# raw-lab/mercat2

Measured on AMD Instinct MI355X. Metric: bases/sec at k=31, 10Mx150bp, higher is better.
Workload: dtype u64

## Files before the change

mercat2_amd/csrc/mk_skmer.hip:

```cpp
#include "mk_skmer_dev.h"
#include <cstdlib>
#include <cstdio>
#include <vector>
#include <type_traits>

#define SK_NKMAX 8
#ifndef SK_HIST_THREADS
#define SK_HIST_THREADS 256
#endif
#ifndef SK_HIST_GRID
#define SK_HIST_GRID 512
#endif
#ifndef SK_SCAT_GRID
#define SK_SCAT_GRID 4096
#endif
#define SK_MAX_P1_LOG2 13
#define SK_MAX_P1 (1 << SK_MAX_P1_LOG2)
#ifndef SK_BUCKET_SYMS
#define SK_BUCKET_SYMS 8192
#endif
#define SK_NOFIT 0xFF000000u

template <int W, class F>
__device__ __forceinline__ void sk_for_each_record(u64 w0, u64 w1, u64 badw, int k, int nkmax, bool canon, F&& emit) {
  const SkRuns r = sk_analyse<W>(w0, w1, sk_valid32(badw, k), canon);
  sk_walk(r, w0, w1, nkmax, canon, emit);
}

__device__ __forceinline__ ulonglong2 sk_make_record(u64 w0, u64 w1, int jstart, int nk, int k) {
  const int s = 2 * jstart;
  u64 hi = (w0 << s) | ((w1 >> 1) >> (63 - s));
  u64 lo = w1 << s;
  const int t = 2 * (nk + k - 1);
  const u64 mh = t >= 64 ? ~0ull : (~0ull << ((64 - t) & 63));
  const u64 ml = t <= 64 ? 0ull : (~0ull << ((128 - t) & 63));
  hi &= mh;
  lo = (lo & ml) | (u64)nk;
  return make_ulonglong2(hi, lo);
}

template <int W, bool CANON>
__global__ __launch_bounds__(SK_HIST_THREADS) void mk_sk_hist_k(const u64* __restrict__ codes, const u64* __restrict__ bad,
                                                                const MkChunkInfo* __restrict__ info, u64* __restrict__ hist,
                                                                u64* __restrict__ khist, int p1_log2, int k, int nkmax,
                                                                size_t nthreads_total, int canon, int sample_log2) {
  extern __shared__ unsigned sk_hist_lds[];
  (void)canon;
  sk_hist_body(sk_hist_lds, sk_hist_lds + (1u << p1_log2), info, hist, p1_log2, nthreads_total, sample_log2,
               [&](size_t t, size_t p0, auto&& tally) {
                 sk_for_each_record<W>(codes[t], codes[t + 1], bad_window(bad, p0), k, nkmax, CANON, tally);
               });
}

#ifndef SK_TU_CANON
__device__ __forceinline__ u64 sk_cap(u64 h, int sample_log2, u64 weight, float sigmas) {
  if (sample_log2 == 0) return h;
  const u64 est = h << sample_log2;
  const float dev = sigmas * __builtin_sqrtf((float)((u64)weight << sample_log2) * (float)est);
  return est + (u64)dev + 1 + (sigmas > 0 ? 16 * weight : 0);
}
__device__ __forceinline__ u64 sk_seg_cap(u64 h, int sample_log2, u64 weight, float sigmas, int nseg) {
  const float est = (float)(h << sample_log2);
  const float var = (float)weight * est * (1.0f / (float)nseg + (float)(1u << sample_log2) / (float)(nseg * nseg));
  return (u64)(est / (float)nseg) + (u64)(sigmas * __builtin_sqrtf(var)) + 1 + (sigmas > 0 ? 4 * weight : 0);
}
__global__ __launch_bounds__(1024) void mk_sk_scan_k(const u64* __restrict__ hist, const u64* __restrict__ khist,
                                                     u64* __restrict__ start, SkCursor* __restrict__ cursor, u64* __restrict__ kstart,
                                                     MkChunkInfo* __restrict__ info, int p1_log2, int sample_log2, int nkmax,
                                                     u64 div, u64 part_cap, u64 surv_cap, float sigmas, int nseg) {
  constexpr int PER = SK_MAX_P1 / 1024;
  __shared__ u64 wsum[16], wksum[16];
  const unsigned p1 = 1u << p1_log2;
  const unsigned per = (p1 + 1023) / 1024;
  const unsigned lo = threadIdx.x * per;
  const int lane = threadIdx.x & 63, wv = threadIdx.x >> 6;
  u64 cap[PER], kcap[PER];
  u64 acc = 0, kacc = 0;
#pragma unroll
  for (int q = 0; q < PER; ++q) {
    const unsigned i = lo + q;
    const bool on = (unsigned)q < per && i < p1;
    const u64 hk = on ? hist[i] : 0ull;
    cap[q] = !on ? 0 : (nseg > 1 ? sk_seg_cap(hk & 0xFFFFFFFFull, sample_log2, SK_R / SK_NKMAX, sigmas, 8)
                                 : sk_cap(hk & 0xFFFFFFFFull, sample_log2, SK_R / SK_NKMAX, sigmas));
    kcap[q] = on ? (sk_cap(hk >> 32, sample_log2, SK_R, sigmas) + div - 1) / div : 0;
    acc += cap[q];
    kacc += kcap[q];
  }
  u64 inc = acc, kinc = kacc;
#pragma unroll
  for (int d = 1; d < 64; d <<= 1) {
    const u64 a = __shfl_up(inc, d), b = __shfl_up(kinc, d);
    if (lane >= d) { inc += a; kinc += b; }
  }
  if (lane == 63) { wsum[wv] = inc; wksum[wv] = kinc; }
  __syncthreads();
  u64 run = inc - acc, krun = kinc - kacc;
  for (int w = 0; w < wv; ++w) { run += wsum[w]; krun += wksum[w]; }
  __shared__ u64 s_total;
  if (threadIdx.x == 1023) {
    const u64 total = run + acc, ktotal = krun + kacc;
    s_total = total;
    const u64 all = nseg > 1 ? 16 * total : total;
    start[(size_t)nseg * p1] = all;
    kstart[p1] = ktotal;
    if (all > part_cap) atomicOr(&info->part_overflow, 1ull);
    if (ktotal > surv_cap) atomicOr(&info->part_overflow, 2ull);
  }
  __shared__ unsigned s_run[SK_MAX_P1];
#pragma unroll
  for (int q = 0; q < PER; ++q) {
    const unsigned i = lo + q;
    if ((unsigned)q < per && i < p1) {
      s_run[i] = (unsigned)run;
      kstart[i] = krun;
      run += cap[q];
      krun += kcap[q];
    }
  }
  __syncthreads();
  const u64 total = s_total;
  for (int x = 0; x < nseg; ++x)
    for (unsigned i = threadIdx.x; i < p1; i += 1024) {
      const u64 at = x < 8 ? (u64)x * total + s_run[i] : 8 * total + 8 * (u64)s_run[i];
      start[(size_t)x * p1 + i] = at;
      cursor[(size_t)x * p1 + i] = (SkCursor)at;
    }
}

#endif

#ifdef MK_STAMP
static __device__ u64 skq_dbg[1024 * 8];
#endif
#define SKQ_CAP 512
#if defined(SK_ABL_COARSE) && !defined(SK_PLAIN_CURSORS)
#error "SK_ABL_COARSE needs -DSK_PLAIN_CURSORS (the ablation's region ends differ from the ones sk_reserve8k checks)"
#endif
#ifndef SKQ_THREADS
#define SKQ_THREADS 512
#endif
#define SKQ_WAVES (SKQ_THREADS / 64)
#define SKQ_WALKED 0xFFFFFFFFu
template <int W, bool CANON, int SKQ_SUBT, int SKQ_QCAP>
__global__ __launch_bounds__(SKQ_THREADS) __attribute__((amdgpu_waves_per_eu(4, 4))) void mk_sk_scatterq_k(const u64* __restrict__ codes, const u64* __restrict__ bad,
                                                         MkChunkInfo* __restrict__ info, const u64* __restrict__ start,
                                                         SkCursor* __restrict__ cursor, ulonglong2* __restrict__ part,
                                                         int p1_log2, int k, int nkmax, size_t ntiles, unsigned qcap, int nseg) {
  SkCursor* const shared_cursor = cursor + ((size_t)8 << p1_log2);
  const u64* const shared_start = start + ((size_t)8 << p1_log2);
  if (nseg > 1) {
    unsigned xcc;
    asm volatile("s_getreg_b32 %0, hwreg(HW_REG_XCC_ID)" : "=s"(xcc));
    const size_t seg = xcc & 7u;
    cursor += seg << p1_log2;
    start += seg << p1_log2;
  }
  __shared__ unsigned lh[SK_MAX_P1];
  __shared__ u64 pk_x[SKQ_SUBT][SKQ_WAVES][65];
  __shared__ unsigned queue[SKQ_SUBT][SKQ_WAVES][SKQ_QCAP];
  __shared__ unsigned s_abort;
  if (threadIdx.x == 0) s_abort = info->part_overflow != 0;
  __syncthreads();
  if (s_abort) return;
  unsigned spilled = 0;
  constexpr int NB = SK_MAX_P1 / SKQ_THREADS;
  const unsigned p1 = 1u << p1_log2;
  const size_t seq_len = info->seq_len;
  const int lane = threadIdx.x & 63;
#define wv sk_wave_id()
  auto sk_wave_id = [&]() { int w = (int)threadIdx.x; asm volatile("" : "+v"(w)); return w >> 6; };
  for (unsigned i = threadIdx.x; i < p1; i += blockDim.x) lh[i] = 0;
  __syncthreads();
  u64 tA = 0, tB = 0, tC = 0, tD = 0, tE = 0, tF = 0, t0 = 0, ntile = 0;
  (void)tA; (void)tB; (void)tC; (void)tD; (void)tE; (void)tF; (void)t0; (void)ntile;
  STAMP(t0);
  for (size_t tile = blockIdx.x; tile < ntiles; tile += gridDim.x) {
    ntile += 1;
    unsigned qn[SKQ_SUBT];
#pragma unroll
    for (int st = 0; st < SKQ_SUBT; ++st) {
      const size_t t = (tile * SKQ_SUBT + st) * SKQ_THREADS + threadIdx.x;
      const size_t p0 = t * SK_R;
      SkRuns runs;
      runs.valid = 0;
      runs.starts = 0;
      runs.pos[0] = runs.pos[1] = runs.pos[2] = runs.pos[3] = 0;
      u64 ww0 = 0, ww1 = 0;
      if (p0 < seq_len) {
        ww0 = codes[t];
        ww1 = codes[t + 1];
        runs = sk_analyse<W>(ww0, ww1, sk_valid32(bad_window(bad, p0), k), CANON);
      } else if (p0 < seq_len + SK_R) {
        ww0 = codes[t];
      }
      pk_x[st][wv][lane] = ww0;
      if (lane == 63) pk_x[st][wv][64] = ww1;
      const unsigned s2 = sk_cut_starts(runs.starts, runs.valid, nkmax);
      const unsigned cnt = __popc(s2);
      const unsigned inc = mk_wave_scan_incl(cnt);
      const unsigned total = mk_wave_last(inc);
      unsigned* const myq = queue[st][wv];
      if (total <= qcap) {
        unsigned todo = s2, at = inc - cnt;
        while (todo) {
          const int j = __ffs(todo) - 1;
          todo &= todo - 1;
          const unsigned stop = (s2 | ~runs.valid) & ~((2u << j) - 1);
          const int nk = (stop ? (__ffs(stop) - 1) : SK_R) - j;
          const u64 pw = j < 10 ? runs.pos[0] : (j < 20 ? runs.pos[1] : (j < 30 ? runs.pos[2] : runs.pos[3]));
          const unsigned best = (unsigned)(pw >> (6 * (j % 10))) & 63u;
          myq[at++] = (unsigned)lane | ((unsigned)j << 6) | ((unsigned)nk << 11) | (best << 16);
        }
        __builtin_amdgcn_fence(__ATOMIC_RELEASE, "wavefront");
        __builtin_amdgcn_wave_barrier();
        __builtin_amdgcn_fence(__ATOMIC_ACQUIRE, "wavefront");
        for (unsigned base = 0; base < total; base += 64) {
          const unsigned i = base + lane;
          if (i < total) {
            const unsigned it = myq[i];
            const u64* const wp = &pk_x[st][wv][it & 63u];
            const unsigned mm = sk_canon_mmer(sk_mmer(wp[0], wp[1], (int)(it >> 16)), CANON);
#ifdef SK_ABL_COARSE
            const unsigned b = sk_bucket(mm, p1_log2) & ~63u;
#else
            const unsigned b = sk_bucket(mm, p1_log2);
#endif
            atomicAdd(&lh[b], 1u);
            myq[i] = (it & 0xFFFFu) | (b << 16);
          }
        }
        qn[st] = total;
      } else {
        if (p0 < seq_len)
          sk_walk(runs, ww0, ww1, nkmax, CANON, [&](int, int, unsigned mm) {
            atomicAdd(&lh[sk_bucket(mm, p1_log2)], 1u);
          });
        qn[st] = SKQ_WALKED;
      }
    }
    STAMP_ADD(tA, t0);
    __syncthreads();
    STAMP_ADD(tB, t0);
    unsigned roff = 0;
    asm volatile("" : "+s"(roff));
    SkCursor* const rcursor = cursor + roff;
    const u64* const rstart = start + roff;
    SkCursor* const rshared_cursor = shared_cursor + roff;
    const u64* const rshared_start = shared_start + roff;
#ifndef SK_PLAIN_CURSORS
    if (p1 == SK_MAX_P1) {
      static_assert(NB % 8 == 0, "sk_reserve8");
#pragma unroll
      for (int h = 0; h < NB; h += 8) {
        unsigned v[8], at[8];
#pragma unroll
        for (int i = 0; i < 8; ++i) v[i] = lh[threadIdx.x + (h + i) * SKQ_THREADS];
        unsigned nofit = sk_reserve8<SKQ_THREADS>(v, rcursor + h * SKQ_THREADS, rstart + h * SKQ_THREADS, SK_NOFIT, at);
        if (nseg > 1 && __any(nofit)) {
          unsigned v2[8], at2[8];
#pragma unroll
          for (int i = 0; i < 8; ++i) {
            v2[i] = at[i] >= SK_NOFIT ? v[i] : 0u;
            const unsigned pad = at[i] >= SK_NOFIT ? at[i] & 0xFFFFFFu : 0u;
            if (pad) {
              const u64 end = rstart[threadIdx.x + (h + i) * SKQ_THREADS + 1];
              for (unsigned q = 0; q < pad; ++q) part[end - pad + q] = make_ulonglong2(0, 0);
            }
          }
          nofit = sk_reserve8<SKQ_THREADS>(v2, rshared_cursor + h * SKQ_THREADS, rshared_start + h * SKQ_THREADS, SK_NOFIT, at2);
#pragma unroll
          for (int i = 0; i < 8; ++i) at[i] = v2[i] ? at2[i] : at[i];
        }
        spilled |= nofit;
#pragma unroll
        for (int i = 0; i < 8; ++i) lh[threadIdx.x + (h + i) * SKQ_THREADS] = at[i];
      }
    } else
#endif
    {
      for (unsigned b = threadIdx.x; b < p1; b += SKQ_THREADS) {
        const unsigned v = lh[b];
        u64 r = v ? (u64)atomicAdd(&rcursor[b], v) : 0ull;
#ifdef SK_ABL_COARSE
        const bool fits = v == 0 || r + v <= rstart[b + 64 < p1 ? b + 64 : p1];
#else
        bool fits = v == 0 || r + v <= rstart[b + 1];
        if (!fits && nseg > 1) {
          for (u64 q = r; q < rstart[b + 1]; ++q) part[q] = make_ulonglong2(0, 0);
          r = (u64)atomicAdd(&rshared_cursor[b], v);
          fits = r + v <= rshared_start[b + 1];
        }
#endif
        spilled |= fits ? 0u : 1u;
        lh[b] = fits ? (unsigned)r : SK_NOFIT;
      }
    }
    STAMP_ADD(tC, t0);
    __syncthreads();
    STAMP_ADD(tD, t0);
#pragma unroll
    for (int st = 0; st < SKQ_SUBT; ++st) {
      if (qn[st] != SKQ_WALKED) {
        const unsigned total = qn[st];
        const unsigned* const myq = queue[st][wv];
        for (unsigned base = 0; base < total; base += 64) {
          const unsigned i = base + lane;
          if (i < total) {
            const unsigned it = myq[i];
            const unsigned at = atomicAdd(&lh[it >> 16], 1u);
            const u64* const wp = &pk_x[st][wv][it & 63u];
            ulonglong2 rec = sk_make_record(wp[0], wp[1], (int)((it >> 6) & 31u), (int)((it >> 11) & 31u), k);
            asm volatile("" : "+v"(rec.x), "+v"(rec.y));
            if (at < SK_NOFIT) part[(size_t)at] = rec;
          }
        }
      } else {
        const size_t t = (tile * SKQ_SUBT + st) * SKQ_THREADS + threadIdx.x;
        const size_t p0 = t * SK_R;
        if (p0 < seq_len) {
          const ulonglong2 w = make_ulonglong2(pk_x[st][wv][lane], pk_x[st][wv][lane + 1]);
          const SkRuns runs = sk_analyse<W>(w.x, w.y, sk_valid32(bad_window(bad, p0), k), CANON);
          sk_walk(runs, w.x, w.y, nkmax, CANON, [&](int jstart, int nk, unsigned mm) {
            const unsigned at = atomicAdd(&lh[sk_bucket(mm, p1_log2)], 1u);
            if (at < SK_NOFIT) part[(size_t)at] = sk_make_record(w.x, w.y, jstart, nk, k);
          });
        }
      }
    }
    STAMP_ADD(tE, t0);
    __syncthreads();
    for (unsigned i = threadIdx.x; i < p1; i += blockDim.x) lh[i] = 0;
    __syncthreads();
    STAMP_ADD(tF, t0);
  }
#ifdef MK_STAMP
  if (threadIdx.x == 0 && blockIdx.x < 1024) { u64* d = skq_dbg + (size_t)blockIdx.x * 8; d[0] = tA; d[1] = tB; d[2] = tC; d[3] = tD; d[4] = tE; d[5] = tF; d[6] = ntile; }
#endif
  if (spilled) atomicOr(&info->part_overflow, 4ull);
}
#undef wv


#ifndef SK_TU_CANON
void mk_launch_sk_scan(mk_ctx* c, const u64* hist, const u64* khist, u64* start, SkCursor* cursor, u64* kstart, int p1_log2,
                       int sample_log2, int nkmax, u64 surv_div, u64 part_cap, u64 surv_cap, float sigmas, int nseg) {
  hipLaunchKernelGGL(mk_sk_scan_k, dim3(1), dim3(1024), 0, c->stream, hist, khist, start, cursor, kstart,
                     (MkChunkInfo*)c->info.p, p1_log2, sample_log2, nkmax, surv_div, part_cap, surv_cap, sigmas, nseg);
}

#endif

template <int W, bool CANON>
static void launch_wc(mk_ctx* c, size_t seq_len, int p1_log2, int nkmax, int sample_log2, u64 surv_div, u64 part_cap, u64 surv_cap,
                     u64* hist, u64* start, SkCursor* cursor, u64* khist, u64* kstart, bool reuse, int nseg) {
  MkChunkInfo* info = (MkChunkInfo*)c->info.p;
  const size_t threads = div_up(seq_len, SK_R);
  const size_t tiles = div_up(div_up(threads, (size_t)1 << sample_log2), SK_HIST_THREADS);
  const size_t hist_grid = sample_log2 ? SK_HIST_GRID / 2 : SK_HIST_GRID;
  if (!reuse) {
    const float sigmas = (float)mk_env_double("MK_SAMPLE_SIGMAS", 6.0);
    hipLaunchKernelGGL((mk_sk_hist_k<W, CANON>), dim3((unsigned)(tiles < hist_grid ? tiles : hist_grid)), dim3(SK_HIST_THREADS),
                       2 * sizeof(unsigned) << p1_log2, c->stream,
                       (const u64*)c->codes.p, (const u64*)c->bad.p, info, hist, khist, p1_log2, c->k, nkmax, threads, c->canonical,
                       sample_log2);
    mk_launch_sk_scan(c, (const u64*)hist, (const u64*)khist, start, cursor, kstart, p1_log2, sample_log2, nkmax, surv_div, part_cap,
                      surv_cap, sigmas, nseg);
  }
  const SkQueueShape shape = sk_queue_shape(c);
  const bool three = shape.three;
  const unsigned qcap = shape.qcap;
  const size_t qtiles = div_up(threads, (size_t)SKQ_THREADS * (three ? 3 : 2));
  const dim3 qgrid((unsigned)(qtiles < SK_SCAT_GRID ? qtiles : SK_SCAT_GRID));
  if (three)
    hipLaunchKernelGGL((mk_sk_scatterq_k<W, CANON, 3, 376>), qgrid, dim3(SKQ_THREADS), 0, c->stream, (const u64*)c->codes.p,
                       (const u64*)c->bad.p, info, (const u64*)start, cursor, (ulonglong2*)c->part.p, p1_log2, c->k, nkmax, qtiles, qcap, nseg);
  else
    hipLaunchKernelGGL((mk_sk_scatterq_k<W, CANON, 2, 512>), qgrid, dim3(SKQ_THREADS), 0, c->stream, (const u64*)c->codes.p,
                       (const u64*)c->bad.p, info, (const u64*)start, cursor, (ulonglong2*)c->part.p, p1_log2, c->k, nkmax, qtiles, qcap, nseg);
#ifdef MK_STAMP
  {
    (void)hipStreamSynchronize(c->stream);
    const unsigned g = qgrid.x;
    std::vector<u64> h(8 * 1024);
    (void)hipMemcpyFromSymbol(h.data(), HIP_SYMBOL(skq_dbg), h.size() * 8);
    double a[7] = {0, 0, 0, 0, 0, 0, 0};
    for (unsigned w = 0; w < g && w < 1024; ++w) for (int q = 0; q < 7; ++q) a[q] += (double)h[w * 8 + q] / g;
    fprintf(stderr, "[stamp scatterq] per WG (wave 0): analyse+list+pass1=%.0f barrier1=%.0f cursors=%.0f barrier2=%.0f pass2=%.0f barrier3+clear=%.0f tiles=%.2f grid=%u\n",
            a[0], a[1], a[2], a[3], a[4], a[5], a[6], g);
  }
#endif
}


template <bool CANON>
static bool sk_partition(int W, mk_ctx* c, size_t seq_len, int p1_log2, int nkmax, int sample_log2, u64 surv_div, u64 part_cap, u64 surv_cap,
                         u64* hist, u64* start, SkCursor* cursor, u64* khist, u64* kstart, bool reuse, int nseg) {
  switch (W) {
#define SK_CASE(W_)                                                                                                      \
  case W_: launch_wc<W_, CANON>(c, seq_len, p1_log2, nkmax, sample_log2, surv_div, part_cap, surv_cap, hist, start, cursor, khist, kstart, reuse, nseg); return true;
    SK_CASE(2) SK_CASE(3) SK_CASE(4) SK_CASE(5) SK_CASE(6) SK_CASE(7)
    SK_CASE(8) SK_CASE(9) SK_CASE(10) SK_CASE(11) SK_CASE(12) SK_CASE(13) SK_CASE(14) SK_CASE(15) SK_CASE(16)
    SK_CASE(17) SK_CASE(18) SK_CASE(19) SK_CASE(20) SK_CASE(21) SK_CASE(22)
#undef SK_CASE
    default: return false;
  }
}

#ifdef SK_TU_CANON
bool mk_sk_partition_canon(int W, mk_ctx* c, size_t seq_len, int p1_log2, int nkmax, int sample_log2, u64 surv_div, u64 part_cap,
                           u64 surv_cap, u64* hist, u64* start, SkCursor* cursor, u64* khist, u64* kstart, bool reuse, int nseg) {
  return sk_partition<true>(W, c, seq_len, p1_log2, nkmax, sample_log2, surv_div, part_cap, surv_cap, hist, start, cursor, khist, kstart, reuse, nseg);
}
#else
bool mk_sk_partition_canon(int W, mk_ctx* c, size_t seq_len, int p1_log2, int nkmax, int sample_log2, u64 surv_div, u64 part_cap,
                           u64 surv_cap, u64* hist, u64* start, SkCursor* cursor, u64* khist, u64* kstart, bool reuse, int nseg);

bool mk_part_inherit(mk_ctx* c, size_t seq_len, int p1_log2, uint64_t min_count, bool sampled, bool exact) {
  if (c->part_cooldown > 0 && !exact) c->part_cooldown -= 1;
  const bool reuse = !exact && sampled && c->part_reuse_ok && !c->part_dirty && c->part_cooldown == 0 &&
                     p1_log2 == c->part_prev_p1 && (unsigned long long)min_count == c->part_prev_minc &&
                     seq_len <= c->part_prev_len + c->part_prev_len / 100 && seq_len >= c->part_prev_len - c->part_prev_len / 50 &&
                     !mk_env_set("MK_NO_REUSE");
  if (reuse) c->st.part_reused += 1;
  c->part_dirty = true;
  if (exact) { c->part_reuse_ok = false; c->part_cooldown = 4; }
  else if (sampled && !reuse) {
    c->part_reuse_ok = true;
    c->part_prev_len = seq_len;
    c->part_prev_p1 = p1_log2;
    c->part_prev_minc = (unsigned long long)min_count;
  } else if (!reuse) c->part_reuse_ok = false;
  return reuse;
}

int sk_p1_log2(size_t seq_len, int max_log2, size_t bucket_syms) {
  int p1_log2 = 8;
  while (p1_log2 < max_log2 && (seq_len >> p1_log2) > bucket_syms) ++p1_log2;
  return p1_log2;
}
int sk_sample_log2(size_t seq_len, bool exact) {
  return !exact && seq_len >= (size_t)mk_env_int("MK_SAMPLE_MIN", (long long)8 << 20) ? 3 : 0;
}
u64 sk_surv_div(uint64_t min_count) { return min_count > 1 ? (u64)min_count : 1; }
size_t sk_surv_cap(size_t seq_len, size_t p1, u64 surv_div, int sample_log2) {
  if (!sample_log2) return seq_len / surv_div + p1 + 64;
  const double L = 1.25 * (double)seq_len, S = (double)(1u << sample_log2), w = (double)SK_R;
  return (size_t)((L + 6.0 * sqrt((double)p1 * S * w * L) + 16.0 * w * (double)p1) / (double)surv_div) + 2 * p1 + 64;
}
SkQueueShape sk_queue_shape(const mk_ctx* c) {
  const long long force_subt = mk_env_int("MK_SKQ_SUBT", 0);
  SkQueueShape q;
  q.three = force_subt == 3 || (force_subt != 2 && c->items_hint > 0 && c->items_hint * 64.0 + 48.0 < 376.0);
  q.qcap = q.three ? 376u : 512u;
  { const long long v = mk_env_int("MK_SKQ_CAP", -1); if (v >= 0 && (unsigned long long)v < q.qcap) q.qcap = (unsigned)v; }
  return q;
}

int mk_launch_count_superkmer(mk_ctx* c, size_t seq_len, uint64_t min_count, bool exact) {
  if (seq_len == 0) return MK_OK;
  const int k = c->k;
  const int p1_log2 = sk_p1_log2(seq_len, SK_MAX_P1_LOG2, SK_BUCKET_SYMS);
  c->p1_log2 = p1_log2;
  const size_t p1 = (size_t)1 << p1_log2;
  int nkmax = 62 - k;
  if (nkmax > SK_NKMAX) nkmax = SK_NKMAX;
  { const long long v = mk_env_int("MK_NKMAX", 0); if (v >= 1 && v <= 31 && v <= 62 - k) nkmax = (int)v; }
  const int sample_log2 = sk_sample_log2(seq_len, exact);
  c->part_sampled = sample_log2 != 0;
  const int nseg = (sample_log2 != 0 && seq_len <= ((size_t)1 << 30) && mk_env_int("MK_XSEG", 1) != 0) ? 9 : 1;
  if (nseg != c->part_nseg) c->part_reuse_ok = false;
  c->part_nseg = nseg;
  const bool reuse = mk_part_inherit(c, seq_len, p1_log2, min_count, sample_log2 != 0, exact);
  int rc;
  if ((rc = mk_buf_reserve(c, c->part_meta, sk_meta_words(p1, SKC_SEG_MAX) * sizeof(u64))) != MK_OK) return rc;
  const size_t part_cap = nseg > 1 ? 2 * seq_len + 64 : seq_len + 64;
  if ((rc = mk_buf_reserve(c, c->part, part_cap * sizeof(ulonglong2))) != MK_OK) return rc;
  const u64 surv_div = sk_surv_div(min_count);
  const size_t surv_cap = sk_surv_cap(seq_len, p1, surv_div, sample_log2);
  if ((rc = mk_buf_reserve(c, c->surv_keys, surv_cap * sizeof(u64))) != MK_OK) return rc;
  if ((rc = mk_buf_reserve(c, c->surv_cnts, surv_cap * sizeof(u64))) != MK_OK) return rc;
  const SkMeta m = sk_meta(c->part_meta.p, p1, nseg);
  if (!reuse) MK_HIP(hipMemsetAsync(m.hist, 0, sk_meta_cleared_words(p1) * sizeof(u64), c->stream));
  mk_prof_begin(c, MK_K_PART);
  if (c->canonical) {
    if (!mk_sk_partition_canon(k - SK_M + 1, c, seq_len, p1_log2, nkmax, sample_log2, surv_div, (u64)part_cap, (u64)surv_cap, m.hist, m.start, m.cursor, m.khist, m.kstart, reuse, nseg)) {
      c->err = "mk_launch_count_superkmer: k out of range";
      return MK_ERR_ARG;
    }
  } else if (!sk_partition<false>(k - SK_M + 1, c, seq_len, p1_log2, nkmax, sample_log2, surv_div, (u64)part_cap, (u64)surv_cap, m.hist, m.start, m.cursor, m.khist, m.kstart, reuse, nseg)) {
    c->err = "mk_launch_count_superkmer: k out of range";
    return MK_ERR_ARG;
  }
  mk_prof_end(c);
  if ((rc = mk_launch_sk_count(c, (const u64*)m.start, m.cursor, (const u64*)m.kstart, m.nsurv, min_count, p1, nseg)) != MK_OK) return rc;
  MK_HIP(hipGetLastError());
  c->surv_regions = 1;
  return MK_OK;
}
#endif
```

mercat2_amd/csrc/mk_skmer_dev.h:

```cpp
#pragma once
#include "mk_common.h"
#include "mk_device.h"

#define SK_M 11
#define SK_MASK ((1u << (2 * SK_M)) - 1)
#define SK_R 32

__device__ __forceinline__ unsigned sk_order_raw(unsigned mm) {
  return __umul24(mm, 0x9277B5u) + 0x2C5A3Du;
}
__device__ __forceinline__ unsigned sk_order_hash(unsigned mm) { return sk_order_raw(mm) & SK_MASK; }
__device__ __forceinline__ unsigned sk_canon_mmer(unsigned mm, bool canon) {
  if (!canon) return mm;
  const unsigned rc = (unsigned)mk_revcomp2((u64)mm, SK_M);
  return rc < mm ? rc : mm;
}
__device__ __forceinline__ unsigned sk_bucket(unsigned mm, int p1_log2) { return (mm * 0xC2B2AE3Du) >> (32 - p1_log2); }

__device__ __forceinline__ unsigned sk_mmer(u64 w0, u64 w1, int q) {
  const u64 a = q < 32 ? w0 : w1, b = q < 32 ? w1 : 0ull;
  const int s = 2 * (q & 31);
  const u64 x = (a << s) | ((b >> 1) >> (63 - s));
  return (unsigned)(x >> (64 - 2 * SK_M));
}

typedef unsigned SkCursor;

#ifndef SK_PLAIN_CURSORS
template <int THREADS>
__device__ __forceinline__ unsigned sk_reserve8(const unsigned (&count)[8], SkCursor* cursor, const u64* start, unsigned nofit,
                                                unsigned (&base)[8]) {
  unsigned r[8];
  u64 lim[8];
  const unsigned voff4 = threadIdx.x * 4u, voff8 = threadIdx.x * 8u;
#pragma unroll
  for (int i = 0; i < 8; ++i) {
    u64 saved;
    r[i] = 0;
    asm volatile(
        "v_cmp_ne_u32 vcc, 0, %3\n\t"
        "s_and_saveexec_b64 %1, vcc\n\t"
        "s_nop 4\n\t"
        "global_atomic_add %0, %2, %3, %4 sc0\n\t"
        "s_mov_b64 exec, %1"
        : "+v"(r[i]), "=&s"(saved)
        : "v"(voff4), "v"(count[i]), "s"(cursor + i * THREADS)
        : "memory", "vcc", "scc");
  }
#pragma unroll
  for (int i = 0; i < 8; ++i)
    asm volatile("s_nop 4\n\tglobal_load_dwordx2 %0, %1, %2 offset:8" : "=&v"(lim[i]) : "v"(voff8), "s"(start + i * THREADS) : "memory");
  asm volatile("s_waitcnt vmcnt(0)"
               : "+v"(r[0]), "+v"(r[1]), "+v"(r[2]), "+v"(r[3]), "+v"(r[4]), "+v"(r[5]), "+v"(r[6]), "+v"(r[7]), "+v"(lim[0]),
                 "+v"(lim[1]), "+v"(lim[2]), "+v"(lim[3]), "+v"(lim[4]), "+v"(lim[5]), "+v"(lim[6]), "+v"(lim[7])
               :
               : "memory");
  unsigned spilled = 0;
#pragma unroll
  for (int i = 0; i < 8; ++i) {
    const bool fits = count[i] == 0 || (u64)r[i] + count[i] <= lim[i];
    spilled |= fits ? 0u : 1u;
    base[i] = fits ? r[i] : nofit | ((u64)r[i] < lim[i] ? (unsigned)(lim[i] - r[i]) : 0u);
  }
  return spilled;
}
#endif

template <int THREADS, int MAX_P1>
__device__ __forceinline__ void sk_reserve_tile(unsigned* count, unsigned* base, SkCursor* cursor, const u64* start, unsigned p1,
                                                unsigned nofit, unsigned& spilled) {
#ifndef SK_PLAIN_CURSORS
  if (p1 == MAX_P1) {
    constexpr int NB = MAX_P1 / THREADS;
    static_assert(NB % 8 == 0, "sk_reserve8");
#pragma unroll
    for (int h = 0; h < NB; h += 8) {
      unsigned v[8], at[8];
#pragma unroll
      for (int i = 0; i < 8; ++i) v[i] = count[threadIdx.x + (h + i) * THREADS];
      spilled |= sk_reserve8<THREADS>(v, cursor + h * THREADS, start + h * THREADS, nofit, at);
#pragma unroll
      for (int i = 0; i < 8; ++i) {
        base[threadIdx.x + (h + i) * THREADS] = at[i];
        if (base != count) count[threadIdx.x + (h + i) * THREADS] = 0;
      }
    }
  } else
#endif
  {
    for (unsigned b = threadIdx.x; b < p1; b += THREADS) {
      const unsigned v = count[b];
      const u64 r = v ? (u64)atomicAdd(&cursor[b], v) : 0ull;
      const bool fits = v == 0 || r + v <= start[b + 1];
      spilled |= fits ? 0u : 1u;
      base[b] = fits ? (unsigned)r : nofit;
      if (base != count) count[b] = 0;
    }
  }
}

__device__ __forceinline__ unsigned sk_valid32(u64 badw, int k) {
  if (badw == 0) return ~0u;
  u64 d = badw;
  int cover = 1;
  while (2 * cover <= k) { d |= d >> cover; cover *= 2; }
  if (cover < k) d |= d >> (k - cover);
  return ~(unsigned)d;
}

struct SkRuns {
  unsigned valid, starts;
  u64 pos[4];
};

template <int W>
__device__ __forceinline__ SkRuns sk_analyse(u64 w0, u64 w1, unsigned valid, bool canon) {
  constexpr int NQ = SK_R + W - 1;
  unsigned ord[NQ];
  {
    unsigned mm = sk_mmer(w0, w1, 0);
#pragma unroll
    for (int q = 0; q < NQ; ++q) {
      if (q) {
        const int pos = q + SK_M - 1;
        const unsigned base = (unsigned)((pos < 32 ? (w0 >> (62 - 2 * pos)) : (w1 >> (62 - 2 * (pos - 32)))) & 3u);
        mm = ((mm << 2) | base) & SK_MASK;
      }
      unsigned h = sk_order_raw(sk_canon_mmer(mm, canon));
      asm("" : "+v"(h));
      ord[q] = (h << 10) | (unsigned)q;
    }
  }
  constexpr int WA = W >= 3 ? 3 : 1, WB = W >= 9 ? 9 : WA;
  if constexpr (W >= 3) {
#pragma unroll
    for (int q = 0; q + 2 < NQ; ++q) ord[q] = min(min(ord[q], ord[q + 1]), ord[q + 2]);
  }
  if constexpr (W >= 9) {
#pragma unroll
    for (int q = 0; q + 8 < NQ; ++q) ord[q] = min(min(ord[q], ord[q + 3]), ord[q + 6]);
  }
  static_assert(W <= 3 * WB, "a third round of minima would be needed");
  SkRuns r;
  r.valid = valid;
  r.starts = 0;
  r.pos[0] = r.pos[1] = r.pos[2] = r.pos[3] = 0;
  unsigned prev_pos = 64;
#pragma unroll
  for (int j = 0; j < SK_R; ++j) {
    const bool ok = (valid >> j) & 1u;
    unsigned best;
    if constexpr (W == WB) best = ord[j];
    else if constexpr (W <= 2 * WB) best = min(ord[j], ord[j + W - WB]);
    else best = min(min(ord[j], ord[j + WB]), ord[j + W - WB]);
    best &= 63u;
    r.starts |= (ok && best != prev_pos) ? (1u << j) : 0u;
    prev_pos = ok ? best : 64u;
    r.pos[j / 10] |= (u64)best << (6 * (j % 10));
  }
  return r;
}

template <class F>
__device__ __forceinline__ void sk_walk(const SkRuns& r, u64 w0, u64 w1, int nkmax, bool canon, F&& emit) {
  unsigned todo = r.starts;
  while (todo) {
    const int j = __ffs(todo) - 1;
    todo &= todo - 1;
    const unsigned stop = (r.starts | ~r.valid) & ~((2u << j) - 1);
    int nk = (stop ? (__ffs(stop) - 1) : SK_R) - j;
    const u64 pw = j < 10 ? r.pos[0] : (j < 20 ? r.pos[1] : (j < 30 ? r.pos[2] : r.pos[3]));
    const unsigned best = (unsigned)(pw >> (6 * (j % 10))) & 63u;
    const unsigned mm = sk_canon_mmer(sk_mmer(w0, w1, (int)best), canon);
    int at = j;
    while (nk > 0) {
      const int take = nk < nkmax ? nk : nkmax;
      emit(at, take, mm);
      at += take;
      nk -= take;
    }
  }
}

__device__ __forceinline__ unsigned sk_cut_starts(unsigned starts, unsigned valid, int nkmax) {
  if (nkmax >= SK_R) return starts;
  const unsigned cont = valid & ~starts;
  unsigned a = cont;
  int len = 1;
  while (2 * len <= nkmax) { a &= a << len; len *= 2; }
  if (len < nkmax) a &= a << (nkmax - len);
  unsigned s2 = starts;
  for (unsigned c = (starts << nkmax) & a; c; c = (c << nkmax) & a) s2 |= c;
  return s2;
}

template <class A>
__device__ __forceinline__ void sk_hist_body(unsigned* lh, unsigned* lk, const MkChunkInfo* __restrict__ info, u64* __restrict__ hist,
                                             int p1_log2, size_t nthreads_total, int sample_log2, A&& analyse) {
  const unsigned p1 = 1u << p1_log2, nthr = blockDim.x;
  for (unsigned i = threadIdx.x; i < p1; i += nthr) { lh[i] = 0; lk[i] = 0; }
  __syncthreads();
  const size_t seq_len = info->seq_len;
  const size_t ngroups = (nthreads_total + ((size_t)1 << sample_log2) - 1) >> sample_log2;
  for (size_t g = (size_t)blockIdx.x * nthr + threadIdx.x; g < ngroups; g += (size_t)gridDim.x * nthr) {
    size_t t = g;
    if (sample_log2) t = (g << sample_log2) + (((unsigned)g * 0x9E3779B1u >> 7) & ((1u << sample_log2) - 1));
    const size_t p0 = t * SK_R;
    if (t >= nthreads_total || p0 >= seq_len) continue;
    analyse(t, p0, [&](int, int nk, unsigned mm) {
      const unsigned b = sk_bucket(mm, p1_log2);
      atomicAdd(&lh[b], 1u);
      atomicAdd(&lk[b], (unsigned)nk);
    });
  }
  __syncthreads();
  for (unsigned b = threadIdx.x; b < p1; b += nthr) {
    const unsigned v = lh[b];
    if (v) atomicAdd(&hist[b], (u64)v | ((u64)lk[b] << 32));
  }
}

#define SKC_SEG_WORDS 20
#define SKC_SEG_MAX 9
__device__ __forceinline__ unsigned skc_seg_at(const unsigned* tab, unsigned j, int nseg) {
  if (nseg == 1) return tab[10] + j;
  const uint4 a = *reinterpret_cast<const uint4*>(tab), b = *reinterpret_cast<const uint4*>(tab + 4);
  const unsigned c = tab[8];
  unsigned x = 0;
#define SKC_SEG_STEP(P) asm("v_cmp_le_u32 vcc, %1, %2\n\tv_addc_co_u32 %0, vcc, 0, %0, vcc" : "+v"(x) : "v"(P), "v"(j) : "vcc")
  SKC_SEG_STEP(a.y); SKC_SEG_STEP(a.z); SKC_SEG_STEP(a.w); SKC_SEG_STEP(b.x); SKC_SEG_STEP(b.y); SKC_SEG_STEP(b.z); SKC_SEG_STEP(b.w);
  SKC_SEG_STEP(c);
#undef SKC_SEG_STEP
  return tab[10 + x] + j;
}
__device__ __forceinline__ void skc_seg_publish(unsigned* tab, unsigned seg_lo, unsigned seg_hi, unsigned seg_end, int nseg) {
  asm volatile("" : "+v"(seg_lo), "+v"(seg_hi), "+v"(seg_end));
  const unsigned x = threadIdx.x & 15u, cnt = x < (unsigned)nseg ? (seg_hi < seg_end ? seg_hi : seg_end) - seg_lo : 0u;
  unsigned inc = cnt;
  inc += (unsigned)__builtin_amdgcn_update_dpp(0, (int)inc, 0x111, 0xf, 0xf, false);
  inc += (unsigned)__builtin_amdgcn_update_dpp(0, (int)inc, 0x112, 0xf, 0xf, false);
  inc += (unsigned)__builtin_amdgcn_update_dpp(0, (int)inc, 0x114, 0xf, 0xf, false);
  inc += (unsigned)__builtin_amdgcn_update_dpp(0, (int)inc, 0x118, 0xf, 0xf, false);
  if (x < SKC_SEG_MAX) {
    tab[x] = inc - cnt;
    tab[10 + x] = seg_lo - (inc - cnt);
  }
  if (x == 15) tab[9] = inc;
}

#ifdef MK_STAMP
#define STAMP(var) { __builtin_amdgcn_sched_barrier(0); unsigned long long t__; asm volatile("s_memtime %0\n\ts_waitcnt lgkmcnt(0)" : "=s"(t__) :: "memory"); __builtin_amdgcn_sched_barrier(0); var = t__; }
#define STAMP_ADD(acc, t0) { unsigned long long t1__; STAMP(t1__); acc += t1__ - t0; t0 = t1__; }
#else
#define STAMP(var)
#define STAMP_ADD(acc, t0)
#endif
```

Measured before the change: 158.2 billion.

## Share overlapping minimizer candidates across lanes via DPP instead of recomputing

Each lane used to hash all SK_R+W-1 m-mer candidates, including the W-1 that overlap the next lane's window. Now each lane hashes only its own 32 candidates and pulls the overlap tail and partial sliding minima from the neighbouring lane with DPP row shifts and readlane. Lane 63 gets its extra candidates from a separately computed cross-wave tail. This removes redundant hashing and min work per thread, at the cost of cross-lane ops. Every lane in a partially valid wave must now take part, so the guards are rewritten around the wave's first position.

Result: no change. 158.1 billion (median of 2 runs) (-0.0%).

```diff
diff --git a/mercat2_amd/csrc/mk_skmer.hip b/mercat2_amd/csrc/mk_skmer.hip
--- a/mercat2_amd/csrc/mk_skmer.hip
+++ b/mercat2_amd/csrc/mk_skmer.hip
@@ -187,13 +187,15 @@
       runs.starts = 0;
       runs.pos[0] = runs.pos[1] = runs.pos[2] = runs.pos[3] = 0;
       u64 ww0 = 0, ww1 = 0;
+      unsigned valid = 0;
       if (p0 < seq_len) {
         ww0 = codes[t];
         ww1 = codes[t + 1];
-        runs = sk_analyse<W>(ww0, ww1, sk_valid32(bad_window(bad, p0), k), CANON);
+        valid = sk_valid32(bad_window(bad, p0), k);
       } else if (p0 < seq_len + SK_R) {
         ww0 = codes[t];
       }
+      if (p0 - (size_t)lane * SK_R < seq_len) runs = sk_analyse_wave<W>(ww0, ww1, valid, CANON);
       pk_x[st][wv][lane] = ww0;
       if (lane == 63) pk_x[st][wv][64] = ww1;
       const unsigned s2 = sk_cut_starts(runs.starts, runs.valid, nkmax);
@@ -318,13 +320,14 @@
       } else {
         const size_t t = (tile * SKQ_SUBT + st) * SKQ_THREADS + threadIdx.x;
         const size_t p0 = t * SK_R;
-        if (p0 < seq_len) {
+        if (p0 - (size_t)lane * SK_R < seq_len) {
           const ulonglong2 w = make_ulonglong2(pk_x[st][wv][lane], pk_x[st][wv][lane + 1]);
-          const SkRuns runs = sk_analyse<W>(w.x, w.y, sk_valid32(bad_window(bad, p0), k), CANON);
-          sk_walk(runs, w.x, w.y, nkmax, CANON, [&](int jstart, int nk, unsigned mm) {
-            const unsigned at = atomicAdd(&lh[sk_bucket(mm, p1_log2)], 1u);
-            if (at < SK_NOFIT) part[(size_t)at] = sk_make_record(w.x, w.y, jstart, nk, k);
-          });
+          const SkRuns runs = sk_analyse_wave<W>(w.x, w.y, p0 < seq_len ? sk_valid32(bad_window(bad, p0), k) : 0u, CANON);
+          if (p0 < seq_len)
+            sk_walk(runs, w.x, w.y, nkmax, CANON, [&](int jstart, int nk, unsigned mm) {
+              const unsigned at = atomicAdd(&lh[sk_bucket(mm, p1_log2)], 1u);
+              if (at < SK_NOFIT) part[(size_t)at] = sk_make_record(w.x, w.y, jstart, nk, k);
+            });
         }
       }
     }
diff --git a/mercat2_amd/csrc/mk_skmer_dev.h b/mercat2_amd/csrc/mk_skmer_dev.h
--- a/mercat2_amd/csrc/mk_skmer_dev.h
+++ b/mercat2_amd/csrc/mk_skmer_dev.h
@@ -113,34 +113,40 @@
   u64 pos[4];
 };
 
+template <int N>
+__device__ __forceinline__ void sk_candidates(u64 w0, u64 w1, bool canon, unsigned* ord) {
+  unsigned mm = sk_mmer(w0, w1, 0);
+#pragma unroll
+  for (int q = 0; q < N; ++q) {
+    if (q) {
+      const int pos = q + SK_M - 1;
+      const unsigned base = (unsigned)((pos < 32 ? (w0 >> (62 - 2 * pos)) : (w1 >> (62 - 2 * (pos - 32)))) & 3u);
+      mm = ((mm << 2) | base) & SK_MASK;
+    }
+    unsigned h = sk_order_raw(sk_canon_mmer(mm, canon));
+    asm("" : "+v"(h));
+    ord[q] = (h << 10) | (unsigned)q;
+  }
+}
+
 template <int W>
-__device__ __forceinline__ SkRuns sk_analyse(u64 w0, u64 w1, unsigned valid, bool canon) {
-  constexpr int NQ = SK_R + W - 1;
-  unsigned ord[NQ];
-  {
-    unsigned mm = sk_mmer(w0, w1, 0);
-#pragma unroll
-    for (int q = 0; q < NQ; ++q) {
-      if (q) {
-        const int pos = q + SK_M - 1;
-        const unsigned base = (unsigned)((pos < 32 ? (w0 >> (62 - 2 * pos)) : (w1 >> (62 - 2 * (pos - 32)))) & 3u);
-        mm = ((mm << 2) | base) & SK_MASK;
-      }
-      unsigned h = sk_order_raw(sk_canon_mmer(mm, canon));
-      asm("" : "+v"(h));
-      ord[q] = (h << 10) | (unsigned)q;
-    }
-  }
-  constexpr int WA = W >= 3 ? 3 : 1, WB = W >= 9 ? 9 : WA;
-  if constexpr (W >= 3) {
-#pragma unroll
-    for (int q = 0; q + 2 < NQ; ++q) ord[q] = min(min(ord[q], ord[q + 1]), ord[q + 2]);
-  }
-  if constexpr (W >= 9) {
-#pragma unroll
-    for (int q = 0; q + 8 < NQ; ++q) ord[q] = min(min(ord[q], ord[q + 3]), ord[q + 6]);
-  }
-  static_assert(W <= 3 * WB, "a third round of minima would be needed");
+struct SkNet {
+  static constexpr int NQ = SK_R + W - 1;
+  static constexpr int WA = W >= 3 ? 3 : 1, WB = W >= 9 ? 9 : WA;
+  static_assert(W >= 1 && W <= 3 * WB, "a third round of minima would be needed");
+};
+template <int N, int STEP>
+__device__ __forceinline__ void sk_min_round(unsigned* ord) {
+#pragma unroll
+  for (int q = 0; q < N; ++q) {
+    unsigned m = min(min(ord[q], ord[q + STEP]), ord[q + 2 * STEP]);
+    asm("" : "+v"(m));
+    ord[q] = m;
+  }
+}
+template <int W>
+__device__ __forceinline__ SkRuns sk_runs_of(const unsigned* ord, unsigned valid) {
+  constexpr int WB = SkNet<W>::WB;
   SkRuns r;
   r.valid = valid;
   r.starts = 0;
@@ -159,6 +165,59 @@
     r.pos[j / 10] |= (u64)best << (6 * (j % 10));
   }
   return r;
+}
+
+template <int W>
+__device__ __forceinline__ SkRuns sk_analyse(u64 w0, u64 w1, unsigned valid, bool canon) {
+  constexpr int NQ = SkNet<W>::NQ;
+  unsigned ord[NQ];
+  sk_candidates<NQ>(w0, w1, canon, ord);
+  if constexpr (W >= 3) sk_min_round<NQ - 2, 1>(ord);
+  if constexpr (W >= 9) sk_min_round<NQ - 8, 3>(ord);
+  return sk_runs_of<W>(ord, valid);
+}
+
+__device__ __forceinline__ unsigned sk_wave_shl(unsigned v, int n) {
+  for (int i = 0; i < n; ++i) v = (unsigned)__builtin_amdgcn_update_dpp(0, (int)v, 0x130, 0xf, 0xf, true);
+  return v;
+}
+template <int E>
+__device__ __forceinline__ void sk_take_above(unsigned* ord, unsigned over, unsigned last, unsigned r32) {
+#pragma unroll
+  for (int i = 0; i < E; ++i) {
+    const unsigned nb = (unsigned)__builtin_amdgcn_update_dpp(0, (int)ord[i], 0x130, 0xf, 0xf, true) + r32;
+    const unsigned xo = (unsigned)__builtin_amdgcn_readlane((int)over, i);
+    ord[SK_R + i] = (xo & last) | (nb & ~last);
+  }
+}
+template <int W>
+__device__ __forceinline__ SkRuns sk_analyse_wave(u64 w0, u64 w1, unsigned valid, bool canon) {
+  static_assert(W - 2 + SK_M <= 32 && SK_R + W - 2 <= 63, "sk_analyse_wave");
+  constexpr int E0 = W >= 3 ? 2 : W - 1, E1 = W >= 9 ? 6 : W - 3, E2 = W - 9;
+  constexpr int EMAX = E2 > E1 ? (E2 > E0 ? E2 : E0) : (E1 > E0 ? E1 : E0);
+  unsigned ord[SK_R + EMAX];
+  sk_candidates<SK_R>(w0, w1, canon, ord);
+  const int lane = (int)(threadIdx.x & 63u);
+  const u64 xw = (u64)(unsigned)__builtin_amdgcn_readlane((int)(unsigned)(w1 >> 32), 63) << 32 |
+                 (u64)(unsigned)__builtin_amdgcn_readlane((int)(unsigned)w1, 63);
+  const int ql = lane < W - 1 ? lane : 0;
+  unsigned hx = sk_order_raw(sk_canon_mmer((unsigned)(xw >> (64 - 2 * SK_M - 2 * ql)) & SK_MASK, canon));
+  asm("" : "+v"(hx));
+  unsigned over = (hx << 10) | (unsigned)(SK_R + ql);
+  unsigned last = lane == 63 ? ~0u : 0u, r32 = SK_R;
+  asm("" : "+v"(last), "+v"(r32));
+  sk_take_above<E0>(ord, over, last, r32);
+  if constexpr (W >= 3) {
+    sk_min_round<SK_R, 1>(ord);
+    over = min(min(over, sk_wave_shl(over, 1)), sk_wave_shl(over, 2));
+    sk_take_above<E1>(ord, over, last, r32);
+  }
+  if constexpr (W >= 9) {
+    sk_min_round<SK_R, 3>(ord);
+    over = min(min(over, sk_wave_shl(over, 3)), sk_wave_shl(over, 6));
+    sk_take_above<E2>(ord, over, last, r32);
+  }
+  return sk_runs_of<W>(ord, valid);
 }
 
 template <class F>
```
